# zyt334/AdaFace

Measured on AMD Instinct MI355X. Metric: 512x512 images/sec @ 50 DDIM steps, batch 8, higher is better.
Workload: dtype bf16

## Files before the change

### adaface_amd/csrc/af_conv_gemm.hip

```cpp
#include "af_kernels.h"

#include <cstdlib>
#include <cstring>
#include <mutex>
#include <type_traits>

template <int BM, int BN> struct TileCfg {
  static constexpr int XR = BM / 32, WR = BN / 32;
  static constexpr int WM = BM / 2, WN = BN / 2;
  static constexpr int MI = WM / 32, NI = WN / 32;
  static constexpr int TILE_BYTES = (BM + BN) * 128;
  static constexpr int EPI_LD = BN + 4;
  static constexpr int EPI_BYTES = BM * EPI_LD * 4;
  static constexpr int LDS_BYTES = (2 * TILE_BYTES > EPI_BYTES) ? 2 * TILE_BYTES : EPI_BYTES;
};

__device__ __forceinline__ void lds_dma16(__amdgpu_buffer_rsrc_t rs, char* lds_base, unsigned voffset, unsigned soffset) {
#if defined(__HIP_DEVICE_COMPILE__)
  __builtin_amdgcn_raw_ptr_buffer_load_lds(rs, (__attribute__((address_space(3))) void*)lds_base, 16, voffset, soffset,
                                           0, 0);
#endif
}

__device__ __forceinline__ void tile_coords(int wg, int nwg, int ntm, int ntn, int gm, int& tm, int& tn) {
// ... 1081 lines not shown
  __builtin_amdgcn_s_barrier();
  if (g == 1) __builtin_amdgcn_s_barrier();
  }
  auto dphase = [&](int t) {
    if (g == 0) {
      if (t + 1 < KT) { stage(w0); wait_keep1(); } else pp_wait_vm<0>();
    } else {
      if (t + 2 < KT) stage(w1);
    }
    __builtin_amdgcn_s_barrier();
  };
  auto cend = [&](int t) {
    if (g == 1) { if (t + 2 < KT) wait_keep1(); else pp_wait_vm<0>(); }
    __builtin_amdgcn_s_barrier();
    const int tmp = rd; rd = w0; w0 = w1; w1 = tmp;
  };
  if constexpr (MG) {
  } else if constexpr (NS) {
    auto tile1 = [&](int t, auto& xc, auto& xp) {
      dphase(t);
      __builtin_amdgcn_s_setprio(1);
      cphase8(rd, xc, xp, std::false_type{}, 0, StageCtx{});
      __builtin_amdgcn_s_setprio(0);
      cend(t);
    };
    int t = 0;
    for (; t + 1 < KT; t += 2) {
      tile1(t, xa8, xb8);
      tile1(t + 1, xb8, xa8);
    }
    if (KT & 1) tile1(t, xa8, xb8);
    if (KT & 1) {
#pragma unroll
      for (int j = 0; j < MI; ++j) mfma8(acc[NI - 1][j], w8[NI - 1], xa8[j], wsc8[FP8 ? NI - 1 : 0]);
    } else {
#pragma unroll
      for (int j = 0; j < MI; ++j) mfma8(acc[NI - 1][j], w8[NI - 1], xb8[j], wsc8[FP8 ? NI - 1 : 0]);
    }
  } else {
    for (int t = 0; t < KT; ++t) {
      dphase(t);
      __builtin_amdgcn_s_setprio(1);
      half(rd, U0, U1);
      pp_wait_lgkm0();
      half(rd, U1, U0);
      pp_wait_lgkm0();
      __builtin_amdgcn_s_setprio(0);
      cend(t);
    }
#pragma unroll
    for (int i = 0; i < NI; ++i)
#pragma unroll
      for (int j = 0; j < MI; ++j)
        acc[i][j] = __builtin_amdgcn_mfma_f32_16x16x32_bf16(__builtin_bit_cast(bf16x8, wf[i][1]),
                                                            __builtin_bit_cast(bf16x8, xf[j][1]), acc[i][j], 0, 0, 0);
  }
  if constexpr (!MG) { if (g == 0) __builtin_amdgcn_s_barrier(); }
  if constexpr (NS) load_bias();

  pp_epilogue<BN, LNMODE>(p, acc, bias_r, ln_cs, ln_mu, ln_rs, smem, tid, lane, g, wq, m0, n0, tn, zk);
}

#ifdef AF_LAB_ABLATE
__device__ unsigned long long g_lab_stamps[2048 * 5];
extern "C" int af_lab_stamps(unsigned long long* out, int n) {
  return hipMemcpyFromSymbol(out, HIP_SYMBOL(g_lab_stamps), sizeof(unsigned long long) * (size_t)n) == hipSuccess ? 0 : -1;
}
__device__ __forceinline__ unsigned long long lab_now() {
  unsigned long long t;
  __builtin_amdgcn_sched_barrier(0);
  asm volatile("s_memrealtime %0\n\ts_waitcnt lgkmcnt(0)" : "=s"(t)::"memory");
  __builtin_amdgcn_sched_barrier(0);
  return t;
}
#endif
struct Halo8Cfg {
  static constexpr int BN = 160;
  static constexpr int HPIX = 400, HBUF = HPIX * 128, WBYTES = BN * 128;
  static constexpr int W_BASE = 2 * HBUF, LDS_BYTES = 2 * HBUF + 3 * WBYTES;
  static constexpr int NHQ = 7;
  static_assert(LDS_BYTES <= 160 * 1024, "LDS budget");
};

__global__ __launch_bounds__(512) void conv3x3_halo8_kernel(const ConvGemmParams p) {
  using C = PpCfg<160>;
  using H = Halo8Cfg;
  typedef bf16 T;
  constexpr int BN = 160, NI = C::NI, MI = C::MI, NHQ = H::NHQ;
  extern __shared__ __attribute__((aligned(1024))) char smem[];
  const int tid = threadIdx.x, lane = tid & 63, wid = __builtin_amdgcn_readfirstlane(tid >> 6);
  const int g = wid >> 2, wq = wid & 3;
  const int ntm = p.M / 256, ntn = p.N / BN;
  int tm, tn;
  tile_coords(blockIdx.x, gridDim.x, ntm, ntn, p.group_m, tm, tn);
  const int m0 = tm * 256, n0 = tn * BN;
  const int zk = blockIdx.z;
  const __amdgpu_buffer_rsrc_t rs_x = __builtin_amdgcn_make_buffer_rsrc(
      const_cast<T*>(reinterpret_cast<const T*>(p.src)), 0, (int)0xFFFFFFF0u, 0x00020000);
  const __amdgpu_buffer_rsrc_t rs_w = __builtin_amdgcn_make_buffer_rsrc(
      const_cast<T*>(reinterpret_cast<const T*>(p.W)), 0, (int)0xFFFFFFF0u, 0x00020000);

  const int KT_all = p.K / 64;
  const int kt_per = (KT_all + p.splitk - 1) / p.splitk;
  const int kt_begin = zk * kt_per;
#ifdef AF_LAB_ABLATE
  const int lab = p.fast_taps >> 4;
  const int KT = (lab & 16) ? 1 : min(KT_all, kt_begin + kt_per) - kt_begin;
#else
  constexpr int lab = 0;
  const int KT = min(KT_all, kt_begin + kt_per) - kt_begin;
#endif
  const int chunk0 = kt_begin / 9;
#ifdef AF_LAB_ABLATE
  unsigned long long st0 = 0, st1 = 0, st2 = 0;
  if (lab & 64) st0 = lab_now();
#endif

  const int Wo = p.Wo, HW = Wo + 2, wsh = p.wo_shift;
  const int R = 256 >> wsh;
  const int HP = (R + 2) * HW;
  const int img = m0 >> p.howo_shift;
  const int y0 = (m0 & (p.Ho * Wo - 1)) >> wsh;
  const int srow = lane >> 3;
  const unsigned dchunk = (unsigned)((lane & 7) ^ srow);
  const unsigned ldcb = (unsigned)p.ldc * 2u;

  unsigned h_off[NHQ];
  const int nhq = (H::HPIX / 8 - 1 - wid) / 8 + 1;
#pragma unroll
  for (int q = 0; q < NHQ; ++q) {
    const int hp = (wid + 8 * q) * 8 + srow;
    const int hy = hp / HW, hx = hp - hy * HW;
    const int iy = y0 - 1 + hy, ix = hx - 1;
    const bool ok = hp < HP && (unsigned)iy < (unsigned)p.Hi && (unsigned)ix < (unsigned)p.Wi;
    h_off[q] = ok ? (unsigned)((long)img * p.src_batch_stride * 2) + (unsigned)((iy >> p.up) * p.Ws + (ix >> p.up)) * ldcb + dchunk * 16u
                  : 0xFFFFFFFFu;
  }
  unsigned w_off[3];
#pragma unroll
  for (int q = 0; q < 3; ++q) {
    const int n = n0 + (wid + 8 * q) * 8 + srow;
    w_off[q] = (n < p.Wrows && (wid + 8 * q) < BN / 8) ? (unsigned)((long)n * p.ldw * 2) + dchunk * 16u : 0xFFFFFFFFu;
  }
  const int nwq = g == 0 ? 3 : 2;

  const unsigned lds0 = (unsigned)(__UINTPTR_TYPE__)((__attribute__((address_space(3))) char*)smem);
  const unsigned fch0 = (unsigned)((lane >> 4) ^ (lane & 7)) * 16u;
  const unsigned fch1 = (unsigned)(((lane >> 4) + 4) ^ (lane & 7)) * 16u;
  const unsigned w_base = (unsigned)((g * C::HN + (lane & 15)) * 128);
  int xhp[MI];
#pragma unroll
  for (int j = 0; j < MI; ++j) {
    const int t = wq * 64 + j * 16 + (lane & 15);
    xhp[j] = (t >> wsh) * HW + (t & (Wo - 1));
  }
  const unsigned qsel = (unsigned)(lane >> 4);

  f32x4 acc[NI][MI];
#pragma unroll
  for (int i = 0; i < NI; ++i)
#pragma unroll
    for (int j = 0; j < MI; ++j) acc[i][j] = f32x4{0.f, 0.f, 0.f, 0.f};
  pp_u32x4 w8[NI][2], xa8[MI][2], xb8[MI][2];
#pragma unroll
  for (int i = 0; i < NI; ++i) w8[i][0] = w8[i][1] = pp_u32x4{0u, 0u, 0u, 0u};
#pragma unroll
  for (int j = 0; j < MI; ++j) xa8[j][0] = xa8[j][1] = xb8[j][0] = xb8[j][1] = pp_u32x4{0u, 0u, 0u, 0u};
  auto mfma2 = [&](f32x4& c, const pp_u32x4 (&wv)[2], const pp_u32x4 (&xv)[2]) {
    if (lab & 4) return;
    c = __builtin_amdgcn_mfma_f32_16x16x32_bf16(__builtin_bit_cast(bf16x8, wv[0]), __builtin_bit_cast(bf16x8, xv[0]), c, 0, 0, 0);
    c = __builtin_amdgcn_mfma_f32_16x16x32_bf16(__builtin_bit_cast(bf16x8, wv[1]), __builtin_bit_cast(bf16x8, xv[1]), c, 0, 0, 0);
    asm volatile("" : "+v"(c));
  };
  auto wait_block = [&](auto nc, pp_u32x4 (&blk)[2]) {
    constexpr int n = decltype(nc)::value;
    asm volatile("s_waitcnt lgkmcnt(%2)" : "+v"(blk[0]), "+v"(blk[1]) : "n"(n) : "memory");
  };

  struct Step { int tap, chunk; };
  bool in_loop = false;
  auto stage_w = [&](auto qc, int wslot, Step st, int live) {
    constexpr int q = decltype(qc)::value;
    if ((lab & 1) && in_loop) return;
    if ((lab & 32) && !in_loop) return;
    const unsigned k0b = (unsigned)(st.tap * p.Cin + st.chunk * 64) * 2u;
    const unsigned a = live ? w_off[q] : 0xFFFFFFFFu;
    lds_dma16(rs_w, smem + H::W_BASE + wslot * H::WBYTES + (wid + 8 * q) * 1024, a, k0b);
  };
  auto stage_h = [&](auto qc, int hbuf, int chunk, int live) {
    constexpr int q = decltype(qc)::value;
    if ((lab & 1) && in_loop) return;
    if ((lab & 32) && !in_loop) return;
    const unsigned a = live ? h_off[q] : 0xFFFFFFFFu;
    lds_dma16(rs_x, smem + hbuf * H::HBUF + (wid + 8 * q) * 1024, a, (unsigned)chunk * 128u);
  };
  const int nchunks_all = p.Cin >> 6;
  const int step_end = kt_begin + KT;
  const bool stg = p.pp_stagger != 0;

  auto step = [&](int s_glob, int tap, int hb, int ws, int ws2, pp_u32x4 (&xc)[MI][2], pp_u32x4 (&xp)[MI][2]) {
    constexpr int NB = NI + MI;
    const int chunk = s_glob / 9;
    const int s2 = s_glob + 2;
    Step st2;
    st2.chunk = s2 / 9;
    st2.tap = s2 - st2.chunk * 9;
    const int live_w = s2 < step_end ? 1 : 0;
    const int live_h = ((chunk + 1) * 9 < step_end && chunk + 1 < nchunks_all) ? 1 : 0;
    const int ky = (tap * 11) >> 5, kx = tap - 3 * ky;
    const int tapoff = ky * HW + kx;
    unsigned xa0[MI];
#pragma unroll
    for (int j = 0; j < MI; ++j) {
      const unsigned hp = (unsigned)(xhp[j] + tapoff);
      xa0[j] = lds0 + (unsigned)(hb * H::HBUF) + (hp << 7) + (((qsel ^ hp) & 7u) << 4);
    }
    const unsigned wb0 = lds0 + (unsigned)(H::W_BASE + ws * H::WBYTES) + w_base + fch0;
    const unsigned wb1 = lds0 + (unsigned)(H::W_BASE + ws * H::WBYTES) + w_base + fch1;
    auto rd_block = [&](auto bc) {
      constexpr int bi = decltype(bc)::value;
      if (lab & 2) return;
      if constexpr (bi == 0) {
        w8[0][0] = pp_lds_read128<0>(wb0);
        w8[0][1] = pp_lds_read128<0>(wb1);
      } else if constexpr (bi <= MI) {
        xc[bi - 1][0] = pp_lds_read128<0>(xa0[bi - 1]);
        xc[bi - 1][1] = pp_lds_read128<0>(xa0[bi - 1] ^ 64u);
      } else {
        w8[bi - MI][0] = pp_lds_read128<(bi - MI) * 2048>(wb0);
        w8[bi - MI][1] = pp_lds_read128<(bi - MI) * 2048>(wb1);
      }
    };
    rd_block(std::integral_constant<int, 0>{});
    rd_block(std::integral_constant<int, 1>{});
    __builtin_amdgcn_sched_barrier(0);
    pp_static_for<0, MI * NI>([&](auto mc) {
      constexpr int m = decltype(mc)::value;
      if constexpr (m < MI) {
        mfma2(acc[NI - 1][m], w8[NI - 1], xp[m]);
      } else {
        constexpr int i = (m - MI) / MI, j = (m - MI) % MI;
        constexpr int issued = (2 + m) < NB ? (2 + m) : NB;
        constexpr int need = i == 0 ? 1 + j : (j == 0 ? MI + i : -1);
        if constexpr (need >= 0) {
          std::integral_constant<int, 2 * (issued - need - 1)> cnt;
          if constexpr (i == 0) wait_block(cnt, xc[j]); else wait_block(cnt, w8[i]);
          if constexpr (i == 0 && j == 0) wait_block(cnt, w8[0]);
        }
        mfma2(acc[i][j], w8[i], xc[j]);
      }
      if constexpr (2 + m < NB) rd_block(std::integral_constant<int, 2 + m>{});
      if constexpr (m == MI) { if (g == 0 || !stg) stage_w(std::integral_constant<int, 0>{}, ws2, st2, live_w); }
      if constexpr (m == MI + 1) { if (g == 1 && stg) stage_w(std::integral_constant<int, 0>{}, ws2, st2, live_w); }
      if constexpr (m == MI + 2) { if (g == 0 || !stg) stage_w(std::integral_constant<int, 1>{}, ws2, st2, live_w); }
      if constexpr (m == MI + 3) { if (g == 1 && stg) stage_w(std::integral_constant<int, 1>{}, ws2, st2, live_w); }
      if constexpr (m == MI + 4) { if (g == 0) stage_w(std::integral_constant<int, 2>{}, ws2, st2, live_w); }
      if constexpr (m == MI + 6 || m == MI + 7) {
        if (tap < nhq && (stg ? g == (m - MI - 6) : m == MI + 6)) {
          switch (tap) {
            case 0: stage_h(std::integral_constant<int, 0>{}, hb ^ 1, chunk + 1, live_h); break;
            case 1: stage_h(std::integral_constant<int, 1>{}, hb ^ 1, chunk + 1, live_h); break;
            case 2: stage_h(std::integral_constant<int, 2>{}, hb ^ 1, chunk + 1, live_h); break;
            case 3: stage_h(std::integral_constant<int, 3>{}, hb ^ 1, chunk + 1, live_h); break;
            case 4: stage_h(std::integral_constant<int, 4>{}, hb ^ 1, chunk + 1, live_h); break;
            case 5: stage_h(std::integral_constant<int, 5>{}, hb ^ 1, chunk + 1, live_h); break;
            default: stage_h(std::integral_constant<int, 6>{}, hb ^ 1, chunk + 1, live_h); break;
          }
        }
      }
      __builtin_amdgcn_sched_barrier(0);
    });
    pp_wait_lgkm0();
  };

  pp_static_for<0, NHQ>([&](auto qc) {
    if (decltype(qc)::value < nhq) stage_h(qc, 0, chunk0, 1);
  });
  {
    Step s0{0, chunk0}, s1{1, chunk0};
    stage_w(std::integral_constant<int, 0>{}, 0, s0, 1);
    stage_w(std::integral_constant<int, 1>{}, 0, s0, 1);
    if (g == 0) stage_w(std::integral_constant<int, 2>{}, 0, s0, 1);
    stage_w(std::integral_constant<int, 0>{}, 1, s1, 1);
    stage_w(std::integral_constant<int, 1>{}, 1, s1, 1);
    if (g == 0) stage_w(std::integral_constant<int, 2>{}, 1, s1, 1);
  }
  auto wait_head = [&](int prev_halo) {
    const int n = nwq + prev_halo;
    if (n == 2) pp_wait_vm<2>(); else if (n == 3) pp_wait_vm<3>(); else pp_wait_vm<4>();
  };
  int tap = 0, hb = 0, ws = 0, ws1 = 1, ws2 = 2, s_glob = kt_begin;
  int prev_halo = 0;
  auto one = [&](pp_u32x4 (&xc)[MI][2], pp_u32x4 (&xp)[MI][2]) {
    wait_head(prev_halo);
    __builtin_amdgcn_s_barrier();
    step(s_glob, tap, hb, ws, ws2, xc, xp);
    prev_halo = tap < nhq ? 1 : 0;
    ++s_glob;
    if (++tap == 9) { tap = 0; hb ^= 1; }
    const int t3 = ws; ws = ws1; ws1 = ws2; ws2 = t3;
  };
  int t = 0;
  in_loop = true;
#ifdef AF_LAB_ABLATE
  if (lab & 64) st1 = lab_now();
#endif
  for (; t + 1 < KT; t += 2) {
    one(xa8, xb8);
    one(xb8, xa8);
  }
  if (KT & 1) one(xa8, xb8);
  pp_wait_vm<0>();
  if (KT & 1) {
#pragma unroll
    for (int j = 0; j < MI; ++j) mfma2(acc[NI - 1][j], w8[NI - 1], xa8[j]);
  } else {
#pragma unroll
    for (int j = 0; j < MI; ++j) mfma2(acc[NI - 1][j], w8[NI - 1], xb8[j]);
  }
  __builtin_amdgcn_s_barrier();
#ifdef AF_LAB_ABLATE
  if (lab & 64) st2 = lab_now();
#endif
  if (lab & 8) {
    float sum = 0.f;
#pragma unroll
    for (int i = 0; i < NI; ++i)
#pragma unroll
      for (int j = 0; j < MI; ++j) sum += acc[i][j][0] + acc[i][j][1] + acc[i][j][2] + acc[i][j][3];
    if (sum == 12345.678f) reinterpret_cast<float*>(p.out)[tid] = sum;
    return;
  }

  const int cl = 4 * (lane >> 4);
  float4 bias_r[NI];
#pragma unroll
  for (int i = 0; i < NI; ++i) {
    bias_r[i] = float4{0.f, 0.f, 0.f, 0.f};
    if (p.bias && p.splitk <= 1) bias_r[i] = *reinterpret_cast<const float4*>(p.bias + n0 + g * C::HN + i * 16 + cl);
  }
  float4 ln_cs[1];
  float ln_mu[1], ln_rs[1];
  pp_epilogue<160, 0>(p, acc, bias_r, ln_cs, ln_mu, ln_rs, smem, tid, lane, g, wq, m0, n0, tn, zk);
#ifdef AF_LAB_ABLATE
  if (lab & 64) {
    asm volatile("s_waitcnt vmcnt(0)" ::: "memory");
    __syncthreads();
    const unsigned long long st3 = lab_now();
    unsigned xcc, hwid;
    asm volatile("s_getreg_b32 %0, hwreg(HW_REG_XCC_ID)" : "=s"(xcc));
    asm volatile("s_getreg_b32 %0, hwreg(HW_REG_HW_ID)" : "=s"(hwid));
    if (tid == 0 && blockIdx.x < 2048 && blockIdx.z == 0) {
      unsigned long long* o = g_lab_stamps + (long)blockIdx.x * 5;
      o[0] = st0; o[1] = st1; o[2] = st2; o[3] = st3; o[4] = ((unsigned long long)xcc << 32) | hwid;
    }
  }
#endif
}

template <bool GEGLU, int KC_ = 5, int MJ_ = 2, int D_ = 2> struct RowPanelCfgT {
  static constexpr int KC = KC_, MJ = MJ_, K = KC * 64, D = D_, NS = D_ + 1;
  static constexpr int WROWS = 16 * MJ, BM = 8 * WROWS;
  static constexpr int BN = GEGLU ? 128 : 160;
  static constexpr int WBYTES = BN * 128, WPIECES = BN / 8;
  static constexpr int NIW = BN / 16;
  static constexpr int OCOLS = GEGLU ? BN / 2 : BN;
  static constexpr int OPITCH = OCOLS * 2 + 16, OBYTES = WROWS * OPITCH;
  static constexpr int LDS_BYTES = NS * WBYTES + 8 * OBYTES;
  static constexpr int CPR = OCOLS / 8;
  static constexpr int NST = WROWS * CPR / 64;
  static_assert(LDS_BYTES <= 160 * 1024 && (WROWS * CPR) % 64 == 0 && (MJ * KC == 10 || (MJ == 1 && KC == 20)) && D >= 2 && D <= KC,
                "row-panel LDS / store mapping / 80 (K = 1280, 16 rows per wave: 160) fragment registers / ring depth");
};
typedef RowPanelCfgT<true> RowPanelCfg;

template <bool GEGLU, int LNMODE, bool RES, int KC_ = 5, int MJ_ = 2, int D_ = 2>
__global__ __launch_bounds__(512) void rowpanel_kernel(const ConvGemmParams p) {
  using C = RowPanelCfgT<GEGLU, KC_, MJ_, D_>;
  typedef bf16 T;
  constexpr int KC = C::KC, NIW = C::NIW, MJ = C::MJ, NST = C::NST, CPR = C::CPR, D = C::D, NS = C::NS;
  static_assert(!(GEGLU && (RES || LNMODE == 2)), "GEGLU: plain or LayerNorm-consumer epilogue, no residual");
  extern __shared__ __attribute__((aligned(1024))) char smem[];
  const int tid = threadIdx.x, lane = tid & 63, wid = __builtin_amdgcn_readfirstlane(tid >> 6);
  const int m0 = blockIdx.x * C::BM;
  const int r0 = m0 + wid * C::WROWS;
  const int ntn_all = p.N / C::BN;
  const int nt_begin = (int)((long)blockIdx.y * ntn_all / gridDim.y), nt_end = (int)((long)(blockIdx.y + 1) * ntn_all / gridDim.y);
  const int ntn = nt_end - nt_begin;
  const __amdgpu_buffer_rsrc_t rs_x = __builtin_amdgcn_make_buffer_rsrc(
      const_cast<T*>(reinterpret_cast<const T*>(p.src)), 0, (int)0xFFFFFFF0u, 0x00020000);
  const __amdgpu_buffer_rsrc_t rs_w = __builtin_amdgcn_make_buffer_rsrc(
      const_cast<T*>(reinterpret_cast<const T*>(p.W)), 0, (int)0xFFFFFFF0u, 0x00020000);
  const __amdgpu_buffer_rsrc_t rs_o = __builtin_amdgcn_make_buffer_rsrc(reinterpret_cast<T*>(p.out), 0, (int)0xFFFFFFF0u, 0x00020000);

  float* vecs = reinterpret_cast<float*>(smem + C::LDS_BYTES);
  const int nvcol = ntn * C::BN;
  float4 vb[3], vc[3];
#pragma unroll
  for (int r = 0; r < 3; ++r) {
    const int c4 = tid + 512 * r;
    const int col = nt_begin * C::BN + 4 * c4;
    vb[r] = vc[r] = float4{0.f, 0.f, 0.f, 0.f};
    if (c4 < nvcol / 4) {
      if (p.bias) vb[r] = *reinterpret_cast<const float4*>(p.bias + col);
      if constexpr (LNMODE == 1) vc[r] = *reinterpret_cast<const float4*>(p.ln_colsum + col);
    }
  }

  pp_u32x4 xr[MJ][KC][2];
  unsigned orow[NST];
#pragma unroll
  for (int i = 0; i < NST; ++i) {
    const int c = lane + 64 * i;
    const int row = c / CPR, ch = c - row * CPR;
    const int m = r0 + row;
    orow[i] = m < p.M ? (unsigned)((long)m * p.ldo * 2) + (unsigned)ch * 16u : 0xFFFFFFFFu;
// ... 1099 lines not shown
}
template <int BN> static int launch_pp(const ConvGemmParams& p, hipStream_t stream) {
  const bool gather = !(p.ks == 1 && p.pad == 0);
  dim3 grid(((p.M + 255) / 256) * (p.N / BN), 1, p.splitk > 1 ? p.splitk : 1);
  if (p.ln_stats || p.ln_stats_out) {
    if (gather || p.splitk > 1 || (p.ln_stats && p.ln_stats_out) || (p.ln_stats_out && p.epilogue == AF_EPI_GEGLU)) {
      af_set_error_msg("conv_gemm: LayerNorm-fused launch needs a 1x1 GEMM without split-K");
      return -1;
    }
    return p.ln_stats ? launch_pp_sched<BN, 1, false>(p, grid, stream) : launch_pp_sched<BN, 2, false>(p, grid, stream);
  }
  return gather ? launch_pp_sched<BN, 0, true>(p, grid, stream) : launch_pp_sched<BN, 0, false>(p, grid, stream);
}

template <int BN> static int launch_pp8(const ConvGemmParams& p, hipStream_t stream) {
  const bool gather = !(p.ks == 1 && p.pad == 0);
  dim3 grid(((p.M + 255) / 256) * (p.N / BN), 1, p.splitk > 1 ? p.splitk : 1);
  return gather ? launch_pp_one<BN, 0, true, true, 2>(p, grid, stream) : launch_pp_one<BN, 0, false, true, 2>(p, grid, stream);
}

static int launch_conv_gemm_fp8(ConvGemmParams p, hipStream_t stream, const AfGemmPlan* plan, void* ws) {
  if (p.K % 128 != 0 || p.Cin % 64 != 0 || (p.ks != 1 && p.ks != 3) || p.K < p.ks * p.ks * p.Cin || p.ldw < p.K ||
      p.ldw % 16 != 0 || p.ldc % 16 != 0 || p.ldc < p.Cin || !p.w_scale || p.epilogue == AF_EPI_GEGLU || p.ln_stats || p.ln_stats_out) {
    af_set_error_msg("conv_gemm fp8: K=%d Cin=%d ks=%d ldw=%d ldc=%d (need K%%128==0, Cin%%64==0, ks 1|3, 16-byte pitches, row scales)",
                     p.K, p.Cin, p.ks, p.ldw, p.ldc);
    return -1;
  }
  if (p.N % 4 != 0 || p.ldo % 4 != 0 || (p.residual && p.ldr % 4 != 0) || (p.rowbias && p.ldrb % 4 != 0)) {
    af_set_error_msg("conv_gemm fp8: N/ldo/ldr/ldrb must be multiples of 4 (N=%d ldo=%d)", p.N, p.ldo);
    return -1;
  }
  if (p.M <= 0 || p.N <= 0) return 0;
  {
    const int HoWo = p.Ho * p.Wo > 0 ? p.Ho * p.Wo : 1;
    const double nb = (double)((p.M + HoWo - 1) / HoWo);
    if (nb * (double)p.src_batch_stride >= 4294967280.0 || (double)p.Wrows * p.ldw >= 4294967280.0) {
      af_set_error_msg("conv_gemm fp8: operand exceeds the 4 GB range of the 32-bit gather offsets (split the batch)");
      return -1;
    }
  }
  AfGemmPlan pl = plan ? *plan : af_plan_conv_gemm(p, 1, 2);
  if (pl.tile != 4 && pl.tile != 5) {
    af_set_error_msg("conv_gemm fp8: shape M=%d N=%d K=%d has no fp8 plan (ask af_plan_conv_gemm first)", p.M, p.N, p.K);
    return -1;
  }
  if (pl.splitk > 1 && !ws) pl.splitk = 1;
  p.splitk = pl.splitk;
  p.ws = ws;
  af_set_last_plan(pl);
  g_af_plan_counts[10] += 1;
  if (pl.splitk > 1) g_af_plan_counts[7] += 1;
  {
    auto lg2 = [](int v) { int s = 0; while ((1 << s) < v) ++s; return (v > 0 && (1 << s) == v) ? s : -1; };
    p.howo_shift = lg2(p.Ho * p.Wo);
    p.wo_shift = lg2(p.Wo);
  }
  p.group_m = pl.group_m > 0 ? pl.group_m : 1;
  p.pp_epilogue = g_af_knobs.pp_direct < 0 ? 0 : (g_af_knobs.pp_direct ? 2 : 1);
  if (p.gn_stats_out) {
    if (!af_conv_gn_stats_ok(p, pl, p.gn_cpg)) {
      af_set_error_msg("conv_gemm fp8: GroupNorm partial sums asked of a launch that cannot write them");
      return -1;
    }
    p.pp_epilogue = 2;
    g_af_plan_counts[14] += 1;
  }
  p.k_tap_inner = 1;
  p.fast_taps = g_af_knobs.conv_fast_taps;
  p.pp_stagger = g_af_knobs.pp_stagger;
  AfProfScope prof(AF_K_PP_FP8, stream, 2.0 * p.M * (double)p.N * (p.k_logical ? p.k_logical : p.K),
                   (double)p.M * p.Cin + (double)p.N * p.K + (double)p.M * p.N * 2.0);
  const int rc = pl.tile == 4 ? launch_pp8<128>(p, stream) : launch_pp8<160>(p, stream);
  if (rc) return rc;
  if (p.splitk > 1) {
    const long nq = (long)p.M * (p.N >> 2);
    unsigned blocks = (unsigned)((nq + 255) / 256);
    if (blocks > 4096) blocks = 4096;
    hipLaunchKernelGGL((splitk_reduce_kernel<bf16>), dim3(blocks), dim3(256), 0, stream, p);
    HIP_CHECK_RET(hipGetLastError());
  }
  return 0;
}

static int launch_halo8(const ConvGemmParams& p, hipStream_t stream) {
  static unsigned long long attr_done = 0;
  if (int rc = af_ensure_dynamic_lds(attr_done, reinterpret_cast<const void*>(&conv3x3_halo8_kernel), Halo8Cfg::LDS_BYTES)) return rc;
  dim3 grid((p.M / 256) * (p.N / 160), 1, p.splitk > 1 ? p.splitk : 1);
  hipLaunchKernelGGL(conv3x3_halo8_kernel, grid, dim3(512), Halo8Cfg::LDS_BYTES, stream, p);
  HIP_CHECK_RET(hipGetLastError());
  return 0;
}

template <typename T, int TW, int BN> static int launch_halo(const ConvGemmParams& p, hipStream_t stream) {
  using C = HaloCfg<TW, BN>;
  static unsigned long long attr_done = 0;
  if (int rc = af_ensure_dynamic_lds(attr_done, reinterpret_cast<const void*>(&conv3x3_halo_kernel<T, TW, BN>), C::LDS_BYTES)) return rc;
  dim3 grid((p.M / 128) * ((p.N + BN - 1) / BN), 1, 1);
  hipLaunchKernelGGL((conv3x3_halo_kernel<T, TW, BN>), grid, dim3(256), C::LDS_BYTES, stream, p);
  HIP_CHECK_RET(hipGetLastError());
  return 0;
}

__global__ __launch_bounds__(256) void up_phase4_weights_kernel(const bf16* __restrict__ w3, bf16* __restrict__ w4, long total,
                                                                int rows, int cin, int ldw3) {
  const long idx = (long)blockIdx.x * 256 + threadIdx.x;
  if (idx >= total) return;
  const int n = (int)(idx / cin), c = (int)(idx - (long)n * cin);
  float w[3][3];
#pragma unroll
  for (int ky = 0; ky < 3; ++ky)
#pragma unroll
    for (int kx = 0; kx < 3; ++kx) w[ky][kx] = to_f32<bf16>(w3[(long)n * ldw3 + (ky * 3 + kx) * cin + c]);
  const long ld4 = 4L * cin;
#pragma unroll
  for (int ph = 0; ph < 4; ++ph) {
    const int dy = ph >> 1, dx = ph & 1;
#pragma unroll
    for (int ty = 0; ty < 2; ++ty)
#pragma unroll
      for (int tx = 0; tx < 2; ++tx) {
        const int ylo = ty == 0 ? 0 : (dy == 0 ? 1 : 2), yhi = ty == 0 ? (dy == 0 ? 0 : 1) : 2;
        const int xlo = tx == 0 ? 0 : (dx == 0 ? 1 : 2), xhi = tx == 0 ? (dx == 0 ? 0 : 1) : 2;
        float sum = 0.f;
#pragma unroll
        for (int ky = 0; ky < 3; ++ky)
#pragma unroll
          for (int kx = 0; kx < 3; ++kx)
            if (ky >= ylo && ky <= yhi && kx >= xlo && kx <= xhi) sum += w[ky][kx];
        w4[((long)ph * rows + n) * ld4 + (ty * 2 + tx) * cin + c] = from_f32<bf16>(sum);
      }
  }
}
int af_launch_up_phase4_weights(const void* w3, int rows, int cin, int ldw3, void* w4, hipStream_t stream) {
  const long total = (long)rows * cin;
  if (total <= 0) return 0;
  hipLaunchKernelGGL(up_phase4_weights_kernel, dim3((unsigned)((total + 255) / 256)), dim3(256), 0, stream,
                     reinterpret_cast<const bf16*>(w3), reinterpret_cast<bf16*>(w4), total, rows, cin, ldw3);
  HIP_CHECK_RET(hipGetLastError());
  return 0;
}
static bool up_phase4_ok(const ConvGemmParams& p, int batch) {
  auto pow2 = [](int v) { return v > 0 && (v & (v - 1)) == 0; };
  return p.W_up4 && g_af_knobs.conv_up_phase4 && g_af_knobs.gemm_pp && batch == 1 && p.up == 1 && p.ks == 3 && p.stride == 1 &&
         p.pad == 1 && p.Cin % 64 == 0 && p.ldc >= p.Cin && p.K == 9 * p.Cin && (p.N % 160 == 0 || p.N % 128 == 0) &&
         pow2(p.Hs) && pow2(p.Ws) && p.Ho == 2 * p.Hs && p.Wo == 2 * p.Ws && p.M == (p.M / (p.Ho * p.Wo)) * p.Ho * p.Wo &&
         p.M / 4 >= 1024 && !p.residual && !p.rowbias && !p.ln_stats && !p.ln_stats_out && p.epilogue != AF_EPI_GEGLU &&
         (double)4 * p.Wrows * 4 * p.Cin * 2 < 4294967280.0;
}
static int launch_up_phase4(ConvGemmParams p, hipStream_t stream) {
  auto lg2 = [](int v) { int s = 0; while ((1 << s) < v) ++s; return s; };
  const int bn = p.N % 160 == 0 ? 160 : 128;
  p.W = p.W_up4;
  p.ks = 2; p.up = 0; p.pad = 1;
  p.Hi = p.Ho = p.Hs; p.Wi = p.Wo = p.Ws;
  p.M /= 4;
  p.K = 4 * p.Cin; p.ldw = p.K;
  p.k_logical = p.K;
  p.phase4 = 1;
  p.splitk = 1; p.ws = nullptr;
  p.howo_shift = lg2(p.Ho * p.Wo);
  p.wo_shift = lg2(p.Wo);
  p.pp_epilogue = 2;
  p.k_tap_inner = 1;
  p.fast_taps = 1;
  p.pp_stagger = g_af_knobs.pp_stagger;
  AfGemmPlan pl;
  pl.tile = bn == 160 ? 5 : 4; pl.splitk = 1; pl.ws_bytes = 0; pl.halo_tw = 0; pl.group_m = 1;
  plan_group_m(pl, p);
  p.group_m = pl.group_m > 0 ? pl.group_m : 1;
  af_set_last_plan(pl);
  g_af_plan_counts[13] += 1;
  AfProfScope prof(bn == 160 ? AF_K_PP160_GATHER : AF_K_PP128, stream, 2.0 * p.M * (double)p.N * p.K * 4,
                   ((double)p.M * p.Cin + 4.0 * p.N * p.K + 4.0 * p.M * p.N) * 2);
// ... 224 lines not shown
```

Measured before the change: 10.33.

## Fully unroll the halo8 conv tap loop with compile-time tap, slot and group indices

```diff
diff --git a/adaface_amd/csrc/af_conv_gemm.hip b/adaface_amd/csrc/af_conv_gemm.hip
--- a/adaface_amd/csrc/af_conv_gemm.hip
+++ b/adaface_amd/csrc/af_conv_gemm.hip
@@ -1187,6 +1187,7 @@
   static_assert(LDS_BYTES <= 160 * 1024, "LDS budget");
 };
 
+template <int LABL>
 __global__ __launch_bounds__(512) void conv3x3_halo8_kernel(const ConvGemmParams p) {
   using C = PpCfg<160>;
   using H = Halo8Cfg;
@@ -1200,22 +1201,23 @@
   tile_coords(blockIdx.x, gridDim.x, ntm, ntn, p.group_m, tm, tn);
   const int m0 = tm * 256, n0 = tn * BN;
   const int zk = blockIdx.z;
-  const __amdgpu_buffer_rsrc_t rs_x = __builtin_amdgcn_make_buffer_rsrc(
-      const_cast<T*>(reinterpret_cast<const T*>(p.src)), 0, (int)0xFFFFFFF0u, 0x00020000);
-  const __amdgpu_buffer_rsrc_t rs_w = __builtin_amdgcn_make_buffer_rsrc(
-      const_cast<T*>(reinterpret_cast<const T*>(p.W)), 0, (int)0xFFFFFFF0u, 0x00020000);
+  T* const xsrc = const_cast<T*>(reinterpret_cast<const T*>(p.src));
+  T* const wsrc = const_cast<T*>(reinterpret_cast<const T*>(p.W));
+  const __amdgpu_buffer_rsrc_t rs_x = __builtin_amdgcn_make_buffer_rsrc(xsrc, 0, (int)0xFFFFFFF0u, 0x00020000);
+  const __amdgpu_buffer_rsrc_t rs_w = __builtin_amdgcn_make_buffer_rsrc(wsrc, 0, (int)0xFFFFFFF0u, 0x00020000);
 
   const int KT_all = p.K / 64;
   const int kt_per = (KT_all + p.splitk - 1) / p.splitk;
   const int kt_begin = zk * kt_per;
 #ifdef AF_LAB_ABLATE
   const int lab = p.fast_taps >> 4;
-  const int KT = (lab & 16) ? 1 : min(KT_all, kt_begin + kt_per) - kt_begin;
+  const int KT = (lab & 16) ? 9 : min(KT_all, kt_begin + kt_per) - kt_begin;
 #else
   constexpr int lab = 0;
   const int KT = min(KT_all, kt_begin + kt_per) - kt_begin;
 #endif
   const int chunk0 = kt_begin / 9;
+  const int nch = KT / 9;
 #ifdef AF_LAB_ABLATE
   unsigned long long st0 = 0, st1 = 0, st2 = 0;
   if (lab & 64) st0 = lab_now();
@@ -1241,188 +1243,169 @@
     h_off[q] = ok ? (unsigned)((long)img * p.src_batch_stride * 2) + (unsigned)((iy >> p.up) * p.Ws + (ix >> p.up)) * ldcb + dchunk * 16u
                   : 0xFFFFFFFFu;
   }
+  const unsigned hl6 = (unsigned)(wid < 2 ? 8 * (NHQ - 1) * 1024 : 0);
+  if (wid >= 2) h_off[NHQ - 1] = h_off[0];
   unsigned w_off[3];
 #pragma unroll
   for (int q = 0; q < 3; ++q) {
     const int n = n0 + (wid + 8 * q) * 8 + srow;
     w_off[q] = (n < p.Wrows && (wid + 8 * q) < BN / 8) ? (unsigned)((long)n * p.ldw * 2) + dchunk * 16u : 0xFFFFFFFFu;
   }
-  const int nwq = g == 0 ? 3 : 2;
+  const unsigned cin2 = (unsigned)p.Cin * 2u;
 
   const unsigned lds0 = (unsigned)(__UINTPTR_TYPE__)((__attribute__((address_space(3))) char*)smem);
   const unsigned fch0 = (unsigned)((lane >> 4) ^ (lane & 7)) * 16u;
   const unsigned fch1 = (unsigned)(((lane >> 4) + 4) ^ (lane & 7)) * 16u;
   const unsigned w_base = (unsigned)((g * C::HN + (lane & 15)) * 128);
-  int xhp[MI];
+  const unsigned wrd0 = lds0 + (unsigned)H::W_BASE + w_base + fch0, wrd1 = lds0 + (unsigned)H::W_BASE + w_base + fch1;
+  unsigned xh16[MI];
 #pragma unroll
   for (int j = 0; j < MI; ++j) {
     const int t = wq * 64 + j * 16 + (lane & 15);
-    xhp[j] = (t >> wsh) * HW + (t & (Wo - 1));
-  }
-  const unsigned qsel = (unsigned)(lane >> 4);
+    xh16[j] = (unsigned)((t >> wsh) * HW + (t & (Wo - 1))) << 4;
+  }
+  const unsigned qsel16 = (unsigned)(lane >> 4) << 4;
+  const unsigned hw16 = (unsigned)HW * 16u;
 
   f32x4 acc[NI][MI];
 #pragma unroll
   for (int i = 0; i < NI; ++i)
 #pragma unroll
     for (int j = 0; j < MI; ++j) acc[i][j] = f32x4{0.f, 0.f, 0.f, 0.f};
-  pp_u32x4 w8[NI][2], xa8[MI][2], xb8[MI][2];
+  pp_u32x4 w8[NI][2], xp[MI][2];
 #pragma unroll
   for (int i = 0; i < NI; ++i) w8[i][0] = w8[i][1] = pp_u32x4{0u, 0u, 0u, 0u};
 #pragma unroll
-  for (int j = 0; j < MI; ++j) xa8[j][0] = xa8[j][1] = xb8[j][0] = xb8[j][1] = pp_u32x4{0u, 0u, 0u, 0u};
+  for (int j = 0; j < MI; ++j) xp[j][0] = xp[j][1] = pp_u32x4{0u, 0u, 0u, 0u};
   auto mfma2 = [&](f32x4& c, const pp_u32x4 (&wv)[2], const pp_u32x4 (&xv)[2]) {
-    if (lab & 4) return;
-    c = __builtin_amdgcn_mfma_f32_16x16x32_bf16(__builtin_bit_cast(bf16x8, wv[0]), __builtin_bit_cast(bf16x8, xv[0]), c, 0, 0, 0);
-    c = __builtin_amdgcn_mfma_f32_16x16x32_bf16(__builtin_bit_cast(bf16x8, wv[1]), __builtin_bit_cast(bf16x8, xv[1]), c, 0, 0, 0);
-    asm volatile("" : "+v"(c));
+    if constexpr ((LABL & 4) == 0) {
+      c = __builtin_amdgcn_mfma_f32_16x16x32_bf16(__builtin_bit_cast(bf16x8, wv[0]), __builtin_bit_cast(bf16x8, xv[0]), c, 0, 0, 0);
+      c = __builtin_amdgcn_mfma_f32_16x16x32_bf16(__builtin_bit_cast(bf16x8, wv[1]), __builtin_bit_cast(bf16x8, xv[1]), c, 0, 0, 0);
+      asm volatile("" : "+v"(c));
+    }
   };
   auto wait_block = [&](auto nc, pp_u32x4 (&blk)[2]) {
     constexpr int n = decltype(nc)::value;
     asm volatile("s_waitcnt lgkmcnt(%2)" : "+v"(blk[0]), "+v"(blk[1]) : "n"(n) : "memory");
   };
-
-  struct Step { int tap, chunk; };
-  bool in_loop = false;
-  auto stage_w = [&](auto qc, int wslot, Step st, int live) {
-    constexpr int q = decltype(qc)::value;
-    if ((lab & 1) && in_loop) return;
-    if ((lab & 32) && !in_loop) return;
-    const unsigned k0b = (unsigned)(st.tap * p.Cin + st.chunk * 64) * 2u;
-    const unsigned a = live ? w_off[q] : 0xFFFFFFFFu;
-    lds_dma16(rs_w, smem + H::W_BASE + wslot * H::WBYTES + (wid + 8 * q) * 1024, a, k0b);
-  };
-  auto stage_h = [&](auto qc, int hbuf, int chunk, int live) {
-    constexpr int q = decltype(qc)::value;
-    if ((lab & 1) && in_loop) return;
-    if ((lab & 32) && !in_loop) return;
-    const unsigned a = live ? h_off[q] : 0xFFFFFFFFu;
-    lds_dma16(rs_x, smem + hbuf * H::HBUF + (wid + 8 * q) * 1024, a, (unsigned)chunk * 128u);
-  };
-  const int nchunks_all = p.Cin >> 6;
-  const int step_end = kt_begin + KT;
-  const bool stg = p.pp_stagger != 0;
-
-  auto step = [&](int s_glob, int tap, int hb, int ws, int ws2, pp_u32x4 (&xc)[MI][2], pp_u32x4 (&xp)[MI][2]) {
-    constexpr int NB = NI + MI;
-    const int chunk = s_glob / 9;
-    const int s2 = s_glob + 2;
-    Step st2;
-    st2.chunk = s2 / 9;
-    st2.tap = s2 - st2.chunk * 9;
-    const int live_w = s2 < step_end ? 1 : 0;
-    const int live_h = ((chunk + 1) * 9 < step_end && chunk + 1 < nchunks_all) ? 1 : 0;
-    const int ky = (tap * 11) >> 5, kx = tap - 3 * ky;
-    const int tapoff = ky * HW + kx;
-    unsigned xa0[MI];
-#pragma unroll
-    for (int j = 0; j < MI; ++j) {
-      const unsigned hp = (unsigned)(xhp[j] + tapoff);
-      xa0[j] = lds0 + (unsigned)(hb * H::HBUF) + (hp << 7) + (((qsel ^ hp) & 7u) << 4);
-    }
-    const unsigned wb0 = lds0 + (unsigned)(H::W_BASE + ws * H::WBYTES) + w_base + fch0;
-    const unsigned wb1 = lds0 + (unsigned)(H::W_BASE + ws * H::WBYTES) + w_base + fch1;
-    auto rd_block = [&](auto bc) {
-      constexpr int bi = decltype(bc)::value;
-      if (lab & 2) return;
-      if constexpr (bi == 0) {
-        w8[0][0] = pp_lds_read128<0>(wb0);
-        w8[0][1] = pp_lds_read128<0>(wb1);
-      } else if constexpr (bi <= MI) {
-        xc[bi - 1][0] = pp_lds_read128<0>(xa0[bi - 1]);
-        xc[bi - 1][1] = pp_lds_read128<0>(xa0[bi - 1] ^ 64u);
-      } else {
-        w8[bi - MI][0] = pp_lds_read128<(bi - MI) * 2048>(wb0);
-        w8[bi - MI][1] = pp_lds_read128<(bi - MI) * 2048>(wb1);
-      }
-    };
-    rd_block(std::integral_constant<int, 0>{});
-    rd_block(std::integral_constant<int, 1>{});
-    __builtin_amdgcn_sched_barrier(0);
-    pp_static_for<0, MI * NI>([&](auto mc) {
-      constexpr int m = decltype(mc)::value;
-      if constexpr (m < MI) {
-        mfma2(acc[NI - 1][m], w8[NI - 1], xp[m]);
-      } else {
-        constexpr int i = (m - MI) / MI, j = (m - MI) % MI;
-        constexpr int issued = (2 + m) < NB ? (2 + m) : NB;
-        constexpr int need = i == 0 ? 1 + j : (j == 0 ? MI + i : -1);
-        if constexpr (need >= 0) {
-          std::integral_constant<int, 2 * (issued - need - 1)> cnt;
-          if constexpr (i == 0) wait_block(cnt, xc[j]); else wait_block(cnt, w8[i]);
-          if constexpr (i == 0 && j == 0) wait_block(cnt, w8[0]);
-        }
-        mfma2(acc[i][j], w8[i], xc[j]);
-      }
-      if constexpr (2 + m < NB) rd_block(std::integral_constant<int, 2 + m>{});
-      if constexpr (m == MI) { if (g == 0 || !stg) stage_w(std::integral_constant<int, 0>{}, ws2, st2, live_w); }
-      if constexpr (m == MI + 1) { if (g == 1 && stg) stage_w(std::integral_constant<int, 0>{}, ws2, st2, live_w); }
-      if constexpr (m == MI + 2) { if (g == 0 || !stg) stage_w(std::integral_constant<int, 1>{}, ws2, st2, live_w); }
-      if constexpr (m == MI + 3) { if (g == 1 && stg) stage_w(std::integral_constant<int, 1>{}, ws2, st2, live_w); }
-      if constexpr (m == MI + 4) { if (g == 0) stage_w(std::integral_constant<int, 2>{}, ws2, st2, live_w); }
-      if constexpr (m == MI + 6 || m == MI + 7) {
-        if (tap < nhq && (stg ? g == (m - MI - 6) : m == MI + 6)) {
-          switch (tap) {
-            case 0: stage_h(std::integral_constant<int, 0>{}, hb ^ 1, chunk + 1, live_h); break;
-            case 1: stage_h(std::integral_constant<int, 1>{}, hb ^ 1, chunk + 1, live_h); break;
-            case 2: stage_h(std::integral_constant<int, 2>{}, hb ^ 1, chunk + 1, live_h); break;
-            case 3: stage_h(std::integral_constant<int, 3>{}, hb ^ 1, chunk + 1, live_h); break;
-            case 4: stage_h(std::integral_constant<int, 4>{}, hb ^ 1, chunk + 1, live_h); break;
-            case 5: stage_h(std::integral_constant<int, 5>{}, hb ^ 1, chunk + 1, live_h); break;
-            default: stage_h(std::integral_constant<int, 6>{}, hb ^ 1, chunk + 1, live_h); break;
-          }
-        }
-      }
-      __builtin_amdgcn_sched_barrier(0);
-    });
-    pp_wait_lgkm0();
-  };
-
-  pp_static_for<0, NHQ>([&](auto qc) {
-    if (decltype(qc)::value < nhq) stage_h(qc, 0, chunk0, 1);
-  });
-  {
-    Step s0{0, chunk0}, s1{1, chunk0};
-    stage_w(std::integral_constant<int, 0>{}, 0, s0, 1);
-    stage_w(std::integral_constant<int, 1>{}, 0, s0, 1);
-    if (g == 0) stage_w(std::integral_constant<int, 2>{}, 0, s0, 1);
-    stage_w(std::integral_constant<int, 0>{}, 1, s1, 1);
-    stage_w(std::integral_constant<int, 1>{}, 1, s1, 1);
-    if (g == 0) stage_w(std::integral_constant<int, 2>{}, 1, s1, 1);
-  }
-  auto wait_head = [&](int prev_halo) {
-    const int n = nwq + prev_halo;
-    if (n == 2) pp_wait_vm<2>(); else if (n == 3) pp_wait_vm<3>(); else pp_wait_vm<4>();
-  };
-  int tap = 0, hb = 0, ws = 0, ws1 = 1, ws2 = 2, s_glob = kt_begin;
-  int prev_halo = 0;
-  auto one = [&](pp_u32x4 (&xc)[MI][2], pp_u32x4 (&xp)[MI][2]) {
-    wait_head(prev_halo);
-    __builtin_amdgcn_s_barrier();
-    step(s_glob, tap, hb, ws, ws2, xc, xp);
-    prev_halo = tap < nhq ? 1 : 0;
-    ++s_glob;
-    if (++tap == 9) { tap = 0; hb ^= 1; }
-    const int t3 = ws; ws = ws1; ws1 = ws2; ws2 = t3;
-  };
-  int t = 0;
-  in_loop = true;
+  auto wait_block2 = [&](auto nc, pp_u32x4 (&b0)[2], pp_u32x4 (&b1)[2]) {
+    constexpr int n = decltype(nc)::value;
+    asm volatile("s_waitcnt lgkmcnt(%4)" : "+v"(b0[0]), "+v"(b0[1]), "+v"(b1[0]), "+v"(b1[1]) : "n"(n) : "memory");
+  };
+  auto dma = [&](__amdgpu_buffer_rsrc_t rs, char* dst, unsigned voff, unsigned soff) {
+    if constexpr ((LABL & 1) == 0) lds_dma16(rs, dst, voff, soff);
+  };
+
+  if (!(lab & 32)) {
+    const unsigned kc = (unsigned)chunk0 * 128u;
+#pragma unroll
+    for (int q = 0; q < NHQ; ++q)
+      if (q < nhq) lds_dma16(rs_x, smem + (wid + 8 * q) * 1024, h_off[q], kc);
+#pragma unroll
+    for (int s = 0; s < 2; ++s) {
+      char* const dst = smem + H::W_BASE + s * H::WBYTES + wid * 1024;
+      lds_dma16(rs_w, dst, w_off[0], s * cin2 + kc);
+      lds_dma16(rs_w, dst + 8 * 1024, w_off[1], s * cin2 + kc);
+      if (g == 0) lds_dma16(rs_w, dst + 16 * 1024, w_off[2], s * cin2 + kc);
+    }
+  }
 #ifdef AF_LAB_ABLATE
   if (lab & 64) st1 = lab_now();
 #endif
-  for (; t + 1 < KT; t += 2) {
-    one(xa8, xb8);
-    one(xb8, xa8);
-  }
-  if (KT & 1) one(xa8, xb8);
+
+  auto chunk_loop = [&](auto gc) {
+    constexpr int G = decltype(gc)::value;
+    constexpr int NWQ = G == 0 ? 3 : 2;
+    constexpr int NHT = G == 0 ? 7 : 6;
+    char* const wdst = smem + H::W_BASE + wid * 1024;
+    for (int c = 0; c < nch; ++c) {
+      const unsigned kc = (unsigned)(chunk0 + c) * 128u;
+      const int nrec = c + 1 < nch ? (int)0xFFFFFFF0u : 0;
+      const __amdgpu_buffer_rsrc_t rs_xn = __builtin_amdgcn_make_buffer_rsrc(xsrc, 0, nrec, 0x00020000);
+      const __amdgpu_buffer_rsrc_t rs_wn = __builtin_amdgcn_make_buffer_rsrc(wsrc, 0, nrec, 0x00020000);
+      const unsigned hrd8 = (lds0 + (unsigned)((c & 1) * H::HBUF)) >> 3;
+      char* const hdst = smem + ((c & 1) ^ 1) * H::HBUF + wid * 1024;
+      pp_static_for<0, 9>([&](auto tc) {
+        constexpr int TAP = decltype(tc)::value;
+        constexpr int KY = TAP / 3, KX = TAP % 3, WS = TAP % 3, WS2 = (TAP + 2) % 3, T2 = TAP + 2;
+        constexpr int NB = NI + MI;
+        pp_wait_vm<NWQ + (TAP >= 1 && TAP <= NHT ? 1 : 0)>();
+        __builtin_amdgcn_s_barrier();
+        const unsigned ut = hrd8 + KY * hw16 + KX * 16u;
+        unsigned xa0[MI];
+#pragma unroll
+        for (int j = 0; j < MI; ++j) {
+          const unsigned u = xh16[j] + ut;
+          xa0[j] = (u << 3) | ((u ^ qsel16) & 0x70u);
+        }
+        pp_u32x4 xc[MI][2];
+        if constexpr ((LABL & 2) != 0) {
+#pragma unroll
+          for (int j = 0; j < MI; ++j) xc[j][0] = xc[j][1] = pp_u32x4{0u, 0u, 0u, 0u};
+        }
+        auto rd_block = [&](auto bc) {
+          constexpr int bi = decltype(bc)::value;
+          if constexpr ((LABL & 2) != 0) {
+          } else if constexpr (bi == 0) {
+            w8[0][0] = pp_lds_read128<WS * H::WBYTES>(wrd0);
+            w8[0][1] = pp_lds_read128<WS * H::WBYTES>(wrd1);
+          } else if constexpr (bi <= MI) {
+            xc[bi - 1][0] = pp_lds_read128<0>(xa0[bi - 1]);
+            xc[bi - 1][1] = pp_lds_read128<0>(xa0[bi - 1] ^ 64u);
+          } else {
+            w8[bi - MI][0] = pp_lds_read128<WS * H::WBYTES + (bi - MI) * 2048>(wrd0);
+            w8[bi - MI][1] = pp_lds_read128<WS * H::WBYTES + (bi - MI) * 2048>(wrd1);
+          }
+        };
+        auto stage_w = [&](auto qc) {
+          constexpr int q = decltype(qc)::value;
+          char* const dst = wdst + WS2 * H::WBYTES + 8 * q * 1024;
+          if constexpr (T2 < 9) dma(rs_w, dst, w_off[q], T2 * cin2 + kc);
+          else dma(rs_wn, dst, w_off[q], (T2 - 9) * cin2 + kc + 128u);
+        };
+        auto stage_h = [&]() {
+          if constexpr (TAP < NHT) {
+            if constexpr (TAP < NHQ - 1) dma(rs_xn, hdst + 8 * TAP * 1024, h_off[TAP], kc + 128u);
+            else dma(rs_xn, hdst + hl6, h_off[NHQ - 1], kc + 128u);
+          }
+        };
+        rd_block(std::integral_constant<int, 0>{});
+        rd_block(std::integral_constant<int, 1>{});
+        __builtin_amdgcn_sched_barrier(0);
+        pp_static_for<0, MI * NI>([&](auto mc) {
+          constexpr int m = decltype(mc)::value;
+          if constexpr (m < MI) {
+            mfma2(acc[NI - 1][m], w8[NI - 1], xp[m]);
+          } else {
+            constexpr int i = (m - MI) / MI, j = (m - MI) % MI;
+            constexpr int issued = (2 + m) < NB ? (2 + m) : NB;
+            constexpr int need = i == 0 ? 1 + j : (j == 0 ? MI + i : -1);
+            if constexpr (need >= 0) {
+              std::integral_constant<int, 2 * (issued - need - 1)> cnt;
+              if constexpr (i == 0 && j == 0) wait_block2(cnt, xc[0], w8[0]);
+              else if constexpr (i == 0) wait_block(cnt, xc[j]);
+              else wait_block(cnt, w8[i]);
+            }
+            mfma2(acc[i][j], w8[i], xc[j]);
+          }
+          if constexpr (2 + m < NB) rd_block(std::integral_constant<int, 2 + m>{});
+          if constexpr (m == MI + G) stage_w(std::integral_constant<int, 0>{});
+          if constexpr (m == MI + 2 + G) stage_w(std::integral_constant<int, 1>{});
+          if constexpr (G == 0 && m == MI + 4) stage_w(std::integral_constant<int, 2>{});
+          if constexpr (m == MI + 6 + G) stage_h();
+          __builtin_amdgcn_sched_barrier(0);
+        });
+        pp_wait_lgkm0();
+#pragma unroll
+        for (int j = 0; j < MI; ++j) xp[j][0] = xc[j][0], xp[j][1] = xc[j][1];
+      });
+    }
+  };
+  if (g == 0) chunk_loop(std::integral_constant<int, 0>{});
+  else chunk_loop(std::integral_constant<int, 1>{});
   pp_wait_vm<0>();
-  if (KT & 1) {
-#pragma unroll
-    for (int j = 0; j < MI; ++j) mfma2(acc[NI - 1][j], w8[NI - 1], xa8[j]);
-  } else {
-#pragma unroll
-    for (int j = 0; j < MI; ++j) mfma2(acc[NI - 1][j], w8[NI - 1], xb8[j]);
-  }
+#pragma unroll
+  for (int j = 0; j < MI; ++j) mfma2(acc[NI - 1][j], w8[NI - 1], xp[j]);
   __builtin_amdgcn_s_barrier();
 #ifdef AF_LAB_ABLATE
   if (lab & 64) st2 = lab_now();
@@ -1436,7 +1419,6 @@
     if (sum == 12345.678f) reinterpret_cast<float*>(p.out)[tid] = sum;
     return;
   }
-
   const int cl = 4 * (lane >> 4);
   float4 bias_r[NI];
 #pragma unroll
@@ -2702,13 +2684,33 @@
   return 0;
 }
 
-static int launch_halo8(const ConvGemmParams& p, hipStream_t stream) {
+template <int LABL> static int launch_halo8_lab(const ConvGemmParams& p, hipStream_t stream) {
   static unsigned long long attr_done = 0;
-  if (int rc = af_ensure_dynamic_lds(attr_done, reinterpret_cast<const void*>(&conv3x3_halo8_kernel), Halo8Cfg::LDS_BYTES)) return rc;
+  if (int rc = af_ensure_dynamic_lds(attr_done, reinterpret_cast<const void*>(&conv3x3_halo8_kernel<LABL>), Halo8Cfg::LDS_BYTES))
+    return rc;
   dim3 grid((p.M / 256) * (p.N / 160), 1, p.splitk > 1 ? p.splitk : 1);
-  hipLaunchKernelGGL(conv3x3_halo8_kernel, grid, dim3(512), Halo8Cfg::LDS_BYTES, stream, p);
+  hipLaunchKernelGGL(conv3x3_halo8_kernel<LABL>, grid, dim3(512), Halo8Cfg::LDS_BYTES, stream, p);
   HIP_CHECK_RET(hipGetLastError());
   return 0;
+}
+static int launch_halo8(const ConvGemmParams& p, hipStream_t stream) {
+  if (p.Cin % 64 != 0 || (p.Cin / 64) % (p.splitk > 1 ? p.splitk : 1) != 0) {
+    af_set_error_msg("conv_gemm: halo kernel needs K slices of whole 64-channel chunks (Cin=%d splitk=%d)", p.Cin, p.splitk);
+    return -1;
+  }
+#ifdef AF_LAB_ABLATE
+  switch ((p.fast_taps >> 4) & 7) {
+    case 1: return launch_halo8_lab<1>(p, stream);
+    case 2: return launch_halo8_lab<2>(p, stream);
+    case 3: return launch_halo8_lab<3>(p, stream);
+    case 4: return launch_halo8_lab<4>(p, stream);
+    case 5: return launch_halo8_lab<5>(p, stream);
+    case 6: return launch_halo8_lab<6>(p, stream);
+    case 7: return launch_halo8_lab<7>(p, stream);
+    default: break;
+  }
+#endif
+  return launch_halo8_lab<0>(p, stream);
 }
 
 template <typename T, int TW, int BN> static int launch_halo(const ConvGemmParams& p, hipStream_t stream) {
```

Result: faster. 10.68, median of 6 (+3.5%).
